# Neos-codes/microbeast

Hardware: AMD Instinct MI355X
Metric: env frames/sec (whole node) on 16x16 microRTS (higher is better)
Workload: dtype bf16

## Files before the change

### microbeast_amd/_native.py

```python
from __future__ import annotations

import ctypes
import importlib.util
import os
import sys
import threading
from pathlib import Path

import torch

_LIB = Path(__file__).resolve().parent / "_lib"
_lock = threading.Lock()
_kern = None
_rt = None

c_void_p, c_int, c_int64, c_float = ctypes.c_void_p, ctypes.c_int, ctypes.c_int64, ctypes.c_float

_SIGS = {
    "mbk_multi_copy": [c_void_p, c_int, c_void_p],
    "mbk_comm_standin": [c_void_p, c_void_p, c_int64, c_int, c_int, c_void_p],
    "mbk_row_gather": [c_void_p, c_void_p, c_void_p, c_int, c_int64, c_void_p],
    "mbk_memset": [c_void_p, c_int, c_int64, c_void_p],
    "mbk_masked_cell_fwd": [c_void_p, c_int, c_void_p, c_void_p, c_void_p, c_int, c_int64,
                            c_void_p, c_void_p, c_void_p],
    "mbk_masked_cell_bwd": [c_void_p, c_int, c_void_p, c_void_p, c_void_p, c_void_p, c_int,
                            c_int64, c_void_p, c_int, c_void_p],
    "mbk_row_sum": [c_void_p, c_int64, c_int, c_void_p, c_void_p],
    "mbk_masked_cell_fwd_pbc": [c_void_p, c_int, c_int, c_int, c_void_p, c_void_p, c_void_p,
                                c_int, c_int64, c_void_p, c_void_p, c_void_p],
    "mbk_masked_cell_bwd_pbc": [c_void_p, c_int, c_int, c_int, c_void_p, c_void_p, c_void_p,
                                c_void_p, c_int64, c_void_p, c_void_p],
    "mbk_pconv": [c_void_p, c_void_p],
    "mbk_imgconv": [c_void_p, c_int, c_void_p],
    "mbk_imgwgrad": [c_void_p, c_int, c_void_p],
    "mbk_imgwgrad_parts": [],
    "mbk_cells_nchunk": [c_int],
    "mbk_cells_compact": [c_void_p, c_int, c_int, c_int, c_void_p, c_void_p, c_void_p, c_void_p,
                          c_void_p, c_void_p, c_void_p, c_void_p, c_void_p, c_void_p],
    "mbk_rows_colsum": [c_void_p, c_int, c_int, c_void_p, c_int, c_void_p, c_void_p],
    "mbk_masked_cell_rows_fwd": [c_void_p, c_int, c_void_p, c_void_p, c_int, c_void_p, c_void_p,
                                 c_void_p, c_int, c_void_p, c_void_p, c_void_p],
    "mbk_masked_cell_rows_bwd": [c_void_p, c_int, c_void_p, c_void_p, c_int, c_int, c_void_p,
                                 c_void_p, c_void_p, c_void_p, c_void_p, c_void_p],
    "mbk_pwgrad": [c_void_p, c_void_p],
    "mbk_pwgrad_all": [c_void_p, c_void_p],
    "mbk_pwgrad_all_parts": [c_int, c_int, c_int],
    "mbk_pwgrad_parts": [c_int, c_int, c_int, c_int],
    "mbk_reduce_map": [c_void_p, c_int, c_int64, c_void_p, c_int64, c_void_p, c_void_p],
    "mbk_reduce_inv": [c_void_p, c_int, c_int64, c_void_p, c_int64, c_void_p, c_void_p, c_int64,
                       c_void_p],
    "mbk_ppool_fwd": [c_void_p, c_int, c_int, c_int, c_int, c_void_p, c_void_p, c_void_p],
    "mbk_ppool_bwd": [c_void_p, c_int64, c_int, c_void_p, c_int64, c_int, c_void_p, c_void_p,
                      c_int, c_int, c_int, c_int, c_void_p, c_void_p],
    "mbk_rng_advance": [c_void_p, c_void_p],
    "mbk_vtrace": [c_void_p, c_void_p, c_void_p, c_void_p, c_void_p, c_void_p, c_int, c_int,
                   c_float, c_float, c_float, c_float, c_float, c_float, c_float, c_void_p,
                   c_void_p, c_void_p, c_void_p, c_void_p, c_void_p, c_void_p],
    "mbk_gae": [c_void_p, c_void_p, c_void_p, c_int, c_int, c_float, c_float, c_float, c_int,
                c_void_p, c_void_p, c_void_p, c_void_p, c_void_p],
    "mbk_ppo_loss": [c_void_p, c_void_p, c_void_p, c_void_p, c_void_p, c_void_p, c_void_p,
                     c_void_p, c_int, c_int, c_float, c_float, c_float, c_float, c_float, c_float,
                     c_void_p, c_void_p, c_void_p, c_void_p, c_void_p],
    "mbk_grad_clip_scale": [c_void_p, c_int64, c_float, c_float, c_void_p, c_void_p, c_void_p],
    "mbk_adam": [c_void_p, c_void_p, c_void_p, c_void_p, c_void_p, c_int64, c_float, c_float,
                 c_float, c_float, c_float, c_int64, c_void_p, c_float, c_void_p],
    "mbk_to_bf16": [c_void_p, c_int64, c_void_p, c_void_p],
    "mbk_from_bf16": [c_void_p, c_int64, c_void_p, c_void_p],
    "mbk_conv_fwd": [c_void_p, c_int, c_int, c_int, c_void_p, c_void_p, c_void_p, c_void_p,
                     c_void_p, c_void_p, c_void_p, c_int, c_int, c_int, c_int, c_int, c_int,
                     c_void_p],
    "mbk_conv_fwd_fp8": [c_void_p, c_int, c_int, c_int, c_void_p, c_void_p, c_void_p, c_void_p,
                         c_void_p, c_int, c_int, c_int, c_int, c_int, c_int, c_void_p],
    "mbk_conv_pack_fp8": [c_void_p, c_int, c_void_p],
    "mbk_pool_bwd_idx": [c_void_p, c_void_p, c_int, c_int, c_int, c_int, c_void_p, c_void_p],
    "mbk_conv_wgrad": [c_void_p, c_int, c_int, c_int, c_void_p, c_void_p, c_void_p, c_void_p,
                       c_int, c_int, c_int, c_int, c_int, c_int, c_void_p],
    "mbk_conv_wgrad_parts": [c_int, c_int, c_int, c_int, c_int, c_int, c_int, c_int],
    "mbk_pool_conv_bwd_parts": [c_int, c_int, c_int, c_int, c_int],
    "mbk_pool_conv_bwd": [c_void_p, c_void_p, c_void_p, c_void_p, c_void_p, c_void_p, c_int,
                          c_void_p, c_void_p, c_int, c_int, c_int, c_int, c_int, c_int, c_void_p],
    "mbk_pool_conv_bwd_partial_floats": [c_int, c_int, c_int],
    "mbk_conv_set_grid_cap": [c_int],
    "mbk_set_learner_occupancy": [c_int, c_int],
    "mbk_set_work_queues": [c_int],
    "mbk_set_work_queue_site": [c_int, c_int],
    "mbk_conv0_row_set": [c_int],
    "mbk_fc_wgrad_parts": [c_int, c_int, c_int],
    "mbk_fc_wgrad": [c_void_p, c_void_p, c_int, c_int, c_int, c_void_p, c_int, c_void_p, c_int,
                     c_void_p],
    "mbk_fc_fwd": [c_void_p, c_int, c_void_p, c_void_p, c_void_p, c_void_p, c_int, c_int, c_int,
                   c_void_p, c_void_p, c_void_p],
    "mbk_gemm_nt": [c_void_p, c_void_p, c_void_p, c_void_p, c_int, c_int, c_int, c_int, c_int,
                    c_int, c_int, c_int, c_int, c_void_p],
    "mbk_wgrad_reduce": [c_void_p, c_int, c_int, c_int, c_int, c_void_p, c_void_p, c_int,
                         c_void_p],
    "mbk_wgrad_reduce_batch": [c_void_p, c_int, c_void_p],
    "mbk_pool_bwd": [c_void_p, c_void_p, c_int, c_int, c_int, c_int, c_void_p, c_void_p],
    "mbk_conv_pack": [c_void_p, c_int, c_void_p],
    "mbk_head_compact": [c_void_p, c_int, c_int, c_void_p, c_void_p, c_void_p, c_void_p,
                         c_void_p, c_void_p, c_void_p, c_void_p, c_void_p, c_void_p, c_void_p,
                         c_void_p, c_void_p, c_int, c_void_p, c_void_p, c_void_p, c_void_p],
    "mbk_head_fwd": [c_void_p, c_void_p, c_void_p, c_void_p, c_void_p, c_void_p, c_int,
                     c_void_p, c_void_p, c_void_p, c_void_p, c_void_p, c_void_p, c_int, c_int,
                     c_void_p, c_void_p, c_int, c_void_p],
    "mbk_fc_wgrad_wide_parts": [c_int, c_int, c_int],
    "mbk_fc_wgrad_wide": [c_void_p, c_void_p, c_int, c_int, c_int, c_int, c_void_p, c_int,
                          c_void_p, c_void_p, c_void_p],
    "mbk_head_score": [c_void_p, c_void_p, c_void_p, c_void_p, c_void_p, c_void_p, c_void_p,
                       c_void_p, c_void_p, c_void_p, c_void_p, c_int, c_void_p, c_void_p,
                       c_void_p, c_void_p],
    "mbk_head_pair_rowsum": [c_void_p, c_void_p, c_int, c_int, c_void_p, c_void_p, c_void_p,
                             c_void_p, c_void_p],
    "mbk_head_bwd": [c_void_p, c_void_p, c_void_p, c_void_p, c_void_p, c_void_p, c_void_p,
                     c_void_p, c_void_p, c_void_p, c_void_p, c_void_p, c_void_p, c_void_p,
                     c_void_p, c_int, c_int, c_void_p, c_void_p, c_void_p, c_void_p,
                     c_void_p, c_void_p, c_void_p],
    "mbk_head_dx_gather": [c_void_p, c_void_p, c_void_p, c_int, c_int, c_void_p, c_void_p],
    "mbk_head_dx_value_parts": [c_int],
    "mbk_head_dx_value": [c_void_p, c_void_p, c_void_p, c_int, c_int, c_void_p, c_void_p,
                          c_void_p, c_int, c_void_p, c_void_p, c_int, c_void_p],
    "mbk_head_pack": [c_void_p, c_void_p, c_int, c_void_p, c_void_p, c_void_p, c_void_p],
    "mbk_decode_obs_mask": [c_void_p, c_void_p, c_int, c_int, c_int, c_void_p, c_void_p, c_void_p],
    "mbk_decode_obs_mask_bucket": [c_void_p, c_void_p, c_int, c_int, c_int, c_void_p, c_void_p,
                                   c_void_p, c_void_p, c_void_p, c_void_p, c_void_p],
    "mbk_head_units": [c_void_p, c_int, c_int, c_void_p, c_void_p, c_void_p, c_void_p, c_void_p,
                       c_void_p],
    "mbk_row_sum_rng": [c_void_p, c_int64, c_int, c_void_p, c_void_p, c_void_p],
    "mbk_row_sum_pack": [c_void_p, c_int64, c_int, c_void_p, c_void_p, c_void_p, c_void_p,
                         c_void_p, c_int, c_void_p],
    "mbk_head_fwd_counts": [c_void_p, c_void_p, c_void_p, c_void_p, c_void_p, c_void_p,
# ... 137 lines not shown
```

### microbeast_amd/csrc/kernels/conv.hip

```cpp
#include "../include/mbk_api.h"
#include "common.h"

#include <algorithm>
#include <map>
#include <mutex>

using namespace mbk;

typedef __bf16 bf16x8 __attribute__((ext_vector_type(8)));
typedef short s16x4 __attribute__((ext_vector_type(4)));
typedef float f32x4 __attribute__((ext_vector_type(4)));
typedef __hip_bfloat16 bf16;

namespace {

constexpr int kThreads = 256;

__device__ __forceinline__ float bf2f(bf16 v) { return __bfloat162float(v); }
__device__ __forceinline__ bf16 f2bf(float v) { return __float2bfloat16(v); }

typedef short s16x2 __attribute__((ext_vector_type(2)));
__device__ __forceinline__ uint32_t relu_bf16x2(uint32_t w) {
  s16x2 v = __builtin_bit_cast(s16x2, w);
  v = __builtin_elementwise_max(v, s16x2{0, 0});
// ... 928 lines not shown
      if (tid == 0) ring[(k + 3) & 3] = gen();
      const int r0 = ring[k & 3];
      if (r0 >= nrounds) break;
      round(r0, pf0, k);
      if (tid == 0) ring[(k + 4) & 3] = gen();
      const int r1 = ring[(k + 1) & 3];
      if (r1 >= nrounds) break;
      round(r1, pf1, k + 1);
    }
    if (tid == 0 && __hip_atomic_fetch_add(wq + 1, 1, __ATOMIC_RELAXED, __HIP_MEMORY_SCOPE_AGENT) ==
                        (int)gridDim.x - 1) {
      __hip_atomic_store(wq, 0, __ATOMIC_RELAXED, __HIP_MEMORY_SCOPE_AGENT);
      __hip_atomic_store(wq + 1, 0, __ATOMIC_RELAXED, __HIP_MEMORY_SCOPE_AGENT);
    }
  } else {
    for (int rd = blockIdx.x; rd < nrounds; rd += 2 * gstep) {
      round(rd, pf0, 0);
      if (rd + gstep < nrounds) round(rd + gstep, pf1, 0);
    }
  }
  for (int w = 0; w < kThreads / 64; ++w) {
    if (wave == w) {
#pragma unroll
      for (int mb = 0; mb < MB; ++mb)
#pragma unroll
        for (int nb = 0; nb < NBLK; ++nb)
#pragma unroll
          for (int i = 0; i < 4; ++i) {
            const int co = mb * 16 + 4 * G + i, n = nb * 16 + li;
            float* p = red + co * KTOT + n;
            *p = (w == 0 ? 0.f : *p) + acc[mb][nb][i];
          }
    }
    __syncthreads();
  }
  float* out = a.partial + (size_t)blockIdx.x * (COUT * KTOT + COUT);
  for (int e = tid; e < COUT * KTOT / 4; e += kThreads) ((float4*)out)[e] = ((const float4*)red)[e];
  __syncthreads();
  float* bred = red;
  if (li == 0) {
#pragma unroll
    for (int mb = 0; mb < MB; ++mb)
#pragma unroll
      for (int i = 0; i < 4; ++i) bred[wave * COUT + mb * 16 + 4 * G + i] = accb[mb][i];
  }
  __syncthreads();
  if (tid < COUT) {
    float s = 0.f;
    for (int w = 0; w < kThreads / 64; ++w) s += bred[w * COUT + tid];
    out[COUT * KTOT + tid] = s;
  }
}

__device__ __forceinline__ void wgrad_reduce_cols(const float* __restrict__ partial, int nparts,
                                                  int pps, int split, int colblk,
                                                  float* __restrict__ stage, int cin,
                                                  int cin_real, int cout, float* __restrict__ dw,
                                                  float* __restrict__ db, int accumulate,
                                                  float (*red)[64]) {
  const int ktot = 9 * cin, row = cout * ktot + cout;
  const int col = threadIdx.x & 63, pl = threadIdx.x >> 6;
  const int e = colblk * 64 + col;
  const int p0 = split * pps, p1 = min(nparts, p0 + pps);
  float s = 0.f;
  if (e < row) {
#pragma unroll 4
    for (int p = p0 + pl; p < p1; p += 4) s += partial[(size_t)p * row + e];
  }
  red[pl][col] = s;
  __syncthreads();
  if (pl != 0 || e >= row) return;
  s = red[0][col] + red[1][col] + red[2][col] + red[3][col];
  if (stage) {
    stage[(size_t)split * row + e] = s;
    return;
  }
  if (e < cout * ktot) {
    const int co = e / ktot, r = e - co * ktot, t = r / cin, ci = r - t * cin;
    if (ci >= cin_real) return;
    float* d = dw + ((size_t)co * cin_real + ci) * 9 + t;
    *d = accumulate ? *d + s : s;
  } else if (db) {
    const int co = e - cout * ktot;
    db[co] = accumulate ? db[co] + s : s;
  }
}

__global__ __launch_bounds__(256) void wgrad_reduce_kernel(const float* __restrict__ partial,
                                                           int nparts, int pps,
                                                           float* __restrict__ stage, int cin,
                                                           int cin_real, int cout,
                                                           float* __restrict__ dw,
                                                           float* __restrict__ db, int accumulate) {
  __shared__ float red[4][64];
  wgrad_reduce_cols(partial, nparts, pps, blockIdx.y, blockIdx.x, stage, cin, cin_real, cout, dw,
                    db, accumulate, red);
}

struct MbkReduceJob {
  const float* partial;
  float* dw;
  float* db;
  int nparts, cin, cin_real, cout, accumulate;
};
constexpr int kReducePps = 32;
constexpr int kMaxReduceJobs = 32;
// ... 186 lines not shown
  const int nk = J.cin_real * 9;
  const float* wr = J.w + (size_t)co * nk;
  float m = 0.f;
  for (int e = threadIdx.x; e < nk; e += blockDim.x) m = fmaxf(m, fabsf(wr[e]));
  red[threadIdx.x] = m;
  __syncthreads();
  for (int st = 128; st > 0; st >>= 1) {
    if ((int)threadIdx.x < st) red[threadIdx.x] = fmaxf(red[threadIdx.x], red[threadIdx.x + st]);
    __syncthreads();
  }
  const float amax = red[0];
  int k = 0;
  if (amax > 0.f) {
    k = (int)floorf(log2f(224.f / amax));
    k = max(-30, min(30, k));
  }
  const float sc = ldexpf(1.f, k);
  const int nch = J.cin == 16 ? 5 : 9;
  for (int e = threadIdx.x; e < nch * 32; e += blockDim.x) {
    const int c = e / 32, kk = e % 32;
    int tap, ci;
    if (J.cin == 16) { tap = 2 * c + kk / 16; ci = kk % 16; }
    else { tap = c; ci = kk; }
    float v = 0.f;
    if (tap < 9 && ci < J.cin_real) v = wr[ci * 9 + tap] * sc;
    v = fminf(fmaxf(v, -448.f), 448.f);
    const int b = __builtin_amdgcn_cvt_pk_fp8_f32(v, 0.f, 0, false);
    J.q[(size_t)co * nch * 32 + e] = (uint8_t)(b & 0xFF);
  }
  if (threadIdx.x == 0) J.scale[co] = ldexpf(1.f, -k);
}

inline size_t fwd_smem(int cin, bool bits, int imgs, int H, int W, int cout, bool pool,
                       bool fp8 = false) {
  (void)bits;
  const int pixb = fp8 ? cin + 8 : cin * 2 + 16;
  size_t t = (((size_t)imgs * (H + 2) * (W + 2) * pixb) + 15) & ~(size_t)15;
  if (pool) t += (size_t)imgs * H * W * (cout + 4) * 2;
  return t;
}

inline size_t wgrad_smem(int cin, int cout, int imgs, int H, int W, bool unpool = false) {
  (void)unpool;
  size_t t = wg_tile_bytes(cin, cout, imgs, H, W, wg_band_w(H, W));
  t += 4096;
  t += 64;
  size_t red = (size_t)cout * 9 * cin * 4;
  return t > red ? t : red;
}

int g_grid_cap = 0;
int g_conv0_row = 1;

int resident_blocks(const void* kfn, size_t sm, int (*occ)(int) = nullptr) {
  static int cus = 0;
  if (!cus) {
    int dev = 0;
    hipGetDevice(&dev);
    hipDeviceGetAttribute(&cus, hipDeviceAttributeMultiprocessorCount, dev);
    if (cus <= 0) cus = 256;
  }
  if (sm > 64 * 1024) hipFuncSetAttribute(kfn, hipFuncAttributeMaxDynamicSharedMemorySize, (int)sm);
  int per = 0;
  if (hipOccupancyMaxActiveBlocksPerMultiprocessor(&per, kfn, kThreads, sm) != hipSuccess || per < 1)
    per = 1;
  int r = cus * (occ ? occ(per) : per);
  if (g_grid_cap > 0 && r > g_grid_cap) r = g_grid_cap;
  return r;
}

int fwd_grid(int ngroups, const void* kfn, size_t sm) {
  const long r = (long)resident_blocks(kfn, sm, mbk_occ_f);
  return (int)std::max(1L, std::min((long)ngroups, r));
}

bool index_math_ok(int imgs, int H, int W) {
  return H > 0 && W > 0 && H * W <= 1024 && (int64_t)imgs * H * W < (int64_t(1) << 22);
}

}

static int conv_fwd_launch(const void* x, int in_bits, int cin, int cout, const void* w,
                           const float* wscale, const float* bias, const void* add,
                           const void* mask_src, void* y, void* y_full, void* pool_idx, int N,
                           int H, int W, int imgs, int relu_in, int pool, bool fp8,
                           hipStream_t stream) {
  if (N <= 0) return 0;
  if (fp8 && !wscale) return (int)hipErrorInvalidValue;
  if (!index_math_ok(imgs, H, W)) return (int)hipErrorInvalidValue;
  ConvFwdArgs a{x, (const bf16*)w, bias, (const bf16*)add, (const bf16*)mask_src, (bf16*)y,
                (bf16*)y_full, (uint8_t*)pool_idx, N, H, W, imgs, relu_in, pool, wscale};
  const size_t sm = fwd_smem(cin, in_bits != 0, imgs, H, W, cout, pool != 0, fp8);
  if (sm > 160 * 1024) return (int)hipErrorInvalidValue;
  const int ngroups = (N + imgs - 1) / imgs;
#define LAUNCH(CI, CO, B)                                                                   \
  do {                                                                                      \
    auto kfn = fp8 ? conv_fwd_kernel<CI, CO, B, true> : conv_fwd_kernel<CI, CO, B, false>;  \
    if (sm > 64 * 1024) hipFuncSetAttribute((const void*)kfn,                               \
                                            hipFuncAttributeMaxDynamicSharedMemorySize, (int)sm); \
    const int grid = fwd_grid(ngroups, (const void*)kfn, sm);                               \
    hipLaunchKernelGGL(kfn, dim3(grid), dim3(kThreads), sm, stream, a);                     \
  } while (0)
  if (in_bits && cout == 16 && W > 16 && W <= 32 && !fp8 && g_conv0_row && !add && !mask_src &&
      !relu_in && kLutBytes + (size_t)kRowImgs * H * W * 16 * 2 <= 160 * 1024) {
    const size_t sm0 = kLutBytes + (pool ? (size_t)kRowImgs * H * W * 16 * 2 : 0);
    const auto kfn = conv0_row_kernel<0, 16, true>;
    const int grid = fwd_grid((N + kRowImgs - 1) / kRowImgs, (const void*)kfn, sm0);
    hipLaunchKernelGGL(kfn, dim3(grid), dim3(kThreads), sm0, stream, a);
    return (int)hipGetLastError();
  }
  if (in_bits && (cout == 16 || cout == 32) && W == 16 && !fp8 && g_conv0_row && !add &&
      !mask_src && !relu_in) {
    const size_t sm0 =
        kLutBytes + (pool ? (size_t)kRowImgs * H * 16 * conv0_ostr(cout, false) * 2 : 0);
    if (sm0 > 160 * 1024) return (int)hipErrorInvalidValue;
    const bool hb = H == 16;
    const auto kfn = cout == 16 ? (hb ? conv0_row16_kernel : conv0_row_kernel<0, 16>)
// ... 64 lines not shown
}
extern "C" int mbk_conv_wgrad_parts(int in_bits, int cin, int cout, int N, int H, int W,
                                    int imgs, int unpool) {
  const size_t sm = wgrad_smem(cin, cout, imgs, H, W, unpool != 0);
  if (sm > 160 * 1024 || !index_math_ok(imgs, H, W)) return -(int)hipErrorInvalidValue;
  const int nrounds = (N + imgs - 1) / imgs;
  int res = 1;
  const void* kq = nullptr;
#define Q(CI, CO, B) kq = wgrad_kfn<CI, CO, B>(H, W, unpool != 0)
  WGRAD_DISPATCH(Q)
#undef Q
  if (!kq) return -(int)hipErrorInvalidValue;
  res = resident_blocks(kq, sm, unpool != 0 && 2 * sm + 80 * 1024 <= 160 * 1024 ? occ_b2 : mbk_occ_b);
  return (int)std::max(1L, std::min((long)nrounds, (long)res));
}

extern "C" int mbk_conv_wgrad(const void* x, int in_bits, int cin, int cout, const void* dy,
                              const void* dp, const void* pidx, float* partial, int nparts,
                              int N, int H, int W, int imgs, int relu_in, hipStream_t stream) {
  const bool unpool = dy == nullptr;
  if (unpool && (!dp || !pidx || imgs > 2)) return (int)hipErrorInvalidValue;
  ConvWgradArgs a{x, (const bf16*)dy, partial, N, H, W, imgs, relu_in, (const bf16*)dp,
                  (const uint8_t*)pidx};
#ifndef MBK_WGRAD_QUEUE
#define MBK_WGRAD_QUEUE 1
#endif
  if (MBK_WGRAD_QUEUE) a.queue = mbk_work_queue(stream, kQueueWgrad);
  const size_t sm = wgrad_smem(cin, cout, imgs, H, W, unpool);
  if (sm > 160 * 1024 || nparts < 1 || !index_math_ok(imgs, H, W))
    return (int)hipErrorInvalidValue;
  dim3 grid(nparts);
#define LAUNCH(CI, CO, B)                                                                   \
  do {                                                                                      \
    const void* kfn = wgrad_kfn<CI, CO, B>(H, W, unpool);                    \
    if (!kfn) return (int)hipErrorInvalidValue;                              \
    if (sm > 64 * 1024)                                                                     \
      hipFuncSetAttribute(kfn, hipFuncAttributeMaxDynamicSharedMemorySize, (int)sm);        \
    void* args[] = {&a};                                                                    \
    hipLaunchKernel(kfn, grid, dim3(kThreads), args, sm, stream);                           \
  } while (0)
  if (in_bits) {
    if (cout == 16) LAUNCH(32, 16, true);
    else if (cout == 32) LAUNCH(32, 32, true);
    else return (int)hipErrorInvalidValue;
  } else if (cin == 16 && cout == 16) LAUNCH(16, 16, false);
  else if (cin == 16 && cout == 32) LAUNCH(16, 32, false);
  else if (cin == 32 && cout == 16) LAUNCH(32, 16, false);
  else if (cin == 32 && cout == 32) LAUNCH(32, 32, false);
  else return (int)hipErrorInvalidValue;
#undef LAUNCH
  return (int)hipGetLastError();
}

extern "C" void mbk_conv_set_grid_cap(int cap) { g_grid_cap = cap; }
extern "C" void mbk_conv0_row_set(int on) { g_conv0_row = on; }

extern "C" int mbk_wgrad_reduce(const float* partial, int nparts, int cin, int cin_real, int cout,
                                float* dw, float* db, int accumulate, hipStream_t stream) {
  const int row = cout * 9 * cin + cout;
  const dim3 cols((row + 63) / 64);
  if (nparts > 2 * kReducePps) {
    const int splits = (nparts + kReducePps - 1) / kReducePps;
    float* stage = (float*)partial + (size_t)nparts * row;
    hipLaunchKernelGGL(wgrad_reduce_kernel, dim3(cols.x, splits), dim3(256), 0, stream, partial,
                       nparts, kReducePps, stage, cin, cin_real, cout, dw, db, accumulate);
    hipLaunchKernelGGL(wgrad_reduce_kernel, dim3(cols.x, 1), dim3(256), 0, stream,
                       (const float*)stage, splits, splits, (float*)nullptr, cin, cin_real, cout,
                       dw, db, accumulate);
  } else {
    hipLaunchKernelGGL(wgrad_reduce_kernel, dim3(cols.x, 1), dim3(256), 0, stream, partial,
                       nparts, nparts, (float*)nullptr, cin, cin_real, cout, dw, db, accumulate);
  }
  return (int)hipGetLastError();
}

extern "C" int mbk_wgrad_reduce_batch(const MbkReduceJob* jobs, int n, hipStream_t stream) {
  for (int j0 = 0; j0 < n; j0 += kMaxReduceJobs) {
    const int nj = std::min(kMaxReduceJobs, n - j0);
    ReduceBatch b{};
    int cols = 1, splits = 1;
    bool two = false;
    for (int i = 0; i < nj; ++i) {
      const MbkReduceJob& J = jobs[j0 + i];
      if (!J.partial || !J.dw || J.nparts < 1 || J.cin < 1 || J.cout < 1 || J.cin_real > J.cin)
        return (int)hipErrorInvalidValue;
      b.j[i] = J;
      const int row = J.cout * 9 * J.cin + J.cout;
      cols = std::max(cols, (row + 63) / 64);
      if (J.nparts > 2 * kReducePps) {
        two = true;
        splits = std::max(splits, (J.nparts + kReducePps - 1) / kReducePps);
      }
    }
    hipLaunchKernelGGL(wgrad_reduce_batch_kernel, dim3(cols, splits, nj), dim3(256), 0, stream,
                       b, 0);
    if (two)
      hipLaunchKernelGGL(wgrad_reduce_batch_kernel, dim3(cols, 1, nj), dim3(256), 0, stream, b, 1);
    const int rc = (int)hipGetLastError();
    if (rc) return rc;
  }
  return 0;
}

extern "C" int mbk_pool_bwd(const void* cfull, const void* dp, int N, int H, int W, int C,
                            void* dc, hipStream_t stream) {
  const size_t tot = (size_t)N * H * W * C;
// ... 115 lines not shown
```

### microbeast_amd/ops/encoder.py

```python
from __future__ import annotations

import ctypes
from dataclasses import dataclass

import torch

from .. import _native as N
from .optim import grad_out


@dataclass
class ConvLayer:
    cin: int
    cin_real: int
    cout: int
    H: int
    W: int
    bits: bool
    relu_in: bool
    pool: bool
    w_off: int = 0
    wb_off: int = -1


class _Job(ctypes.Structure):
    _fields_ = [("w", ctypes.c_void_p), ("fwd", ctypes.c_void_p), ("bwd", ctypes.c_void_p),
                ("cin", ctypes.c_int), ("cin_real", ctypes.c_int), ("cout", ctypes.c_int)]


class _RJob(ctypes.Structure):
    _fields_ = [("partial", ctypes.c_void_p), ("dw", ctypes.c_void_p), ("db", ctypes.c_void_p),
                ("nparts", ctypes.c_int), ("cin", ctypes.c_int), ("cin_real", ctypes.c_int),
                ("cout", ctypes.c_int), ("accumulate", ctypes.c_int)]


class _Job8(ctypes.Structure):
    _fields_ = [("w", ctypes.c_void_p), ("q", ctypes.c_void_p), ("scale", ctypes.c_void_p),
                ("cin", ctypes.c_int), ("cin_real", ctypes.c_int), ("cout", ctypes.c_int)]


def _nch(c: int) -> int:
    return 5 if c == 16 else 9


_PF_FWD = 8 * 256
_PF_WGRAD = 4 * 256
_FWD_LDS = 48 * 1024
_FWD_PIX = 512
_RES32_PIX = 256
_RES32_LDS_KB = 100
_RES32_LDS_KB_SMALL = 150


def _imgs_fwd(layer: ConvLayer, cin: int, cout: int, bits: bool, pool: bool,
              fp8: bool = False) -> int:
    hw = layer.H * layer.W
    epp = 1 if bits else cin // 8
    pixb = (cin + 8) if fp8 else (cin * 2 + 16)
    imgs = max(1, _FWD_PIX // hw)
    while imgs > 1:
        sm = imgs * (layer.H + 2) * (layer.W + 2) * pixb + (imgs * hw * (cout + 4) * 2 if pool else 0)
        if sm <= _FWD_LDS and imgs * hw * epp <= _PF_FWD:
            break
        imgs //= 2
    return imgs


def _imgs_wgrad(layer: ConvLayer, unpool: bool = False, unpool_imgs: int = 2) -> int:
    hw = layer.H * layer.W
    xepp = 1 if layer.bits else layer.cin // 8
    dch = layer.cout // 8
    imgs = max(1, min(_PF_WGRAD // (hw * xepp), _PF_WGRAD // (hw * dch)))
    if layer.W in (8, 16, 24) and layer.H % 4 == 0:
        rbx = (layer.W + 2) * layer.cin * 2 + (32 if layer.cin == 32 else 64)
        rbd = layer.W * layer.cout * 2 + (32 if layer.cout == 32 else 128)
        per = (layer.H + 2) * rbx + (layer.H + (2 if layer.cin > layer.cout else 0)) * rbd
    else:
        per = (layer.H + 2) * (layer.W + 2) * layer.cin * 2 + hw * layer.cout * 2
    if unpool:
        imgs = min(imgs, unpool_imgs)
    lim = (72 if layer.cin > layer.cout else 64) * 1024
    while imgs > 1:
        if imgs * per <= lim:
            break
        imgs //= 2
    return imgs


class HipEncoder:

    def __init__(self, h: int, w: int, planes: int, channels=(16, 32, 32), device=None,
                 fp8: bool = False):
        assert planes <= 32, "bit-plane observations carry at most 32 planes"
        self.layers: list[ConvLayer] = []
        H, W, cin, cin_real, bits = h, w, 32, planes, True
        for co in channels:
            self.layers.append(ConvLayer(cin, cin_real, co, H, W, bits, False, True))
            H, W = (H + 1) // 2, (W + 1) // 2
            for _ in range(4):
                self.layers.append(ConvLayer(co, co, co, H, W, False, True, False))
            cin, cin_real, bits = co, co, False
        self.out_hw = (H, W)
        self.out_c = channels[-1]
        off = boff = 0
        for i, L in enumerate(self.layers):
            L.w_off = off
            off += L.cout * _nch(L.cin) * 32
            if i > 0:
                L.wb_off = boff
                boff += L.cin * _nch(L.cout) * 32
        self.packed_fwd = torch.zeros(off, dtype=torch.bfloat16, device=device)
        self.fused_tail = (tuple(channels) == (16, 32, 32) and self.layers[1].H <= 16
                           and self.layers[1].W <= 16)
        self.fused_res_bwd = True
        self.fused_res_bwd32 = True
        self.fused_res_fwd = True
        self.fused_res_fwd32 = True
        self.fused_stage_fwd = True
        self.fused_pool_fwd4 = True
        self.fused_res_blk32_wave = True
        self.fused_res_bwd32_team = True
        self.fused_pool_wgrad0 = True
        self.wgrad0_imgs = 1
        self.fused_pool_conv_bwd = True
        self.defer_reduce = True
        self._pbufs = {}
        self._rjobs = None
        self.packed_bwd = torch.zeros(max(boff, 1), dtype=torch.bfloat16, device=device)
        self.fp8 = fp8
        self.fused_tail8 = True
        self.packed_fwd8 = torch.zeros(off, dtype=torch.uint8, device=device)
        self.scale8 = torch.zeros(sum(L.cout for L in self.layers), dtype=torch.float32,
                                  device=device)
        self._s_off = []
        so = 0
        for L in self.layers:
            self._s_off.append(so)
            so += L.cout

    def pack(self, weights: list[torch.Tensor], with_bwd: bool) -> None:
        k = N.kernels()
        for c0 in range(0, len(self.layers), 16):
            layers = self.layers[c0:c0 + 16]
            jobs = (_Job * len(layers))()
            for i, (L, wt) in enumerate(zip(layers, weights[c0:c0 + 16])):
                assert wt.dtype == torch.float32 and wt.is_contiguous()
                bwd = ((self.packed_bwd.data_ptr() + 2 * L.wb_off)
                       if (with_bwd and L.wb_off >= 0) else None)
                jobs[i] = _Job(wt.data_ptr(), self.packed_fwd.data_ptr() + 2 * L.w_off, bwd,
                               L.cin, L.cin_real, L.cout)
            N.check(k.mbk_conv_pack(ctypes.cast(jobs, ctypes.c_void_p), len(layers),
                                    N.stream_ptr()), "conv_pack")

    def pack_layer(self, i: int, weight: torch.Tensor, with_bwd: bool = False) -> None:
        L = self.layers[i]
        assert weight.dtype == torch.float32 and weight.is_contiguous()
        bwd = ((self.packed_bwd.data_ptr() + 2 * L.wb_off)
               if (with_bwd and L.wb_off >= 0) else None)
        jobs = (_Job * 1)(_Job(weight.data_ptr(), self.packed_fwd.data_ptr() + 2 * L.w_off, bwd,
                               L.cin, L.cin_real, L.cout))
        N.check(N.kernels().mbk_conv_pack(ctypes.cast(jobs, ctypes.c_void_p), 1, N.stream_ptr()),
                "conv_pack")

    def pack_fp8(self, weights: list[torch.Tensor]) -> None:
        k = N.kernels()
        for c0 in range(0, len(self.layers), 16):
            idx = list(range(c0, min(c0 + 16, len(self.layers))))
            jobs = (_Job8 * len(idx))()
            for j, i in enumerate(idx):
                L, wt = self.layers[i], weights[i]
                assert wt.dtype == torch.float32 and wt.is_contiguous()
                jobs[j] = _Job8(wt.data_ptr(), self.packed_fwd8.data_ptr() + L.w_off,
                                self.scale8.data_ptr() + 4 * self._s_off[i], L.cin, L.cin_real,
                                L.cout)
            N.check(k.mbk_conv_pack_fp8(ctypes.cast(jobs, ctypes.c_void_p), len(idx),
# ... 34 lines not shown
                                 ctypes.cast(bp, ctypes.c_void_p), n, L1.H, L1.W,
                                 y.data_ptr(), N.stream_ptr()), "trunk_tail")
        return y

    def _tail8(self, p: torch.Tensor, bs: list[torch.Tensor]) -> torch.Tensor:
        L1, Ll = self.layers[1], self.layers[-1]
        n = p.shape[0]
        base, sbase = self.packed_fwd8.data_ptr(), self.scale8.data_ptr()
        wp = (ctypes.c_void_p * 14)(*[base + L.w_off for L in self.layers[1:15]])
        sp = (ctypes.c_void_p * 14)(*[sbase + 4 * self._s_off[i] for i in range(1, 15)])
        bp = (ctypes.c_void_p * 14)(*[b.data_ptr() for b in bs[1:15]])
        y = torch.empty(n, Ll.H, Ll.W, Ll.cout, dtype=torch.bfloat16, device=p.device)
        N.check(N.kernels().mbk_trunk_tail_fp8(
            p.data_ptr(), ctypes.cast(wp, ctypes.c_void_p), ctypes.cast(sp, ctypes.c_void_p),
            ctypes.cast(bp, ctypes.c_void_p), n, L1.H, L1.W, y.data_ptr(), N.stream_ptr()),
            "trunk_tail_fp8")
        return y

    def _fwd(self, L: ConvLayer, x, bias, add=None, mask_src=None, y_full=None, dgrad=False,
             pool_idx=None):
        n = x.shape[0]
        if dgrad:
            cin, cout, w = L.cout, L.cin, self.packed_bwd.data_ptr() + 2 * L.wb_off
            H, W = L.H, L.W
            bits, relu, pool = False, False, False
        else:
            cin, cout, w = L.cin, L.cout, self.packed_fwd.data_ptr() + 2 * L.w_off
            H, W, bits, relu, pool = L.H, L.W, L.bits, L.relu_in, L.pool
        Ho, Wo = ((H + 1) // 2, (W + 1) // 2) if pool else (H, W)
        y = torch.empty(n, Ho, Wo, cout, dtype=torch.bfloat16, device=x.device)
        imgs = _imgs_fwd(L, cin, cout, bits, pool)
        N.check(N.kernels().mbk_conv_fwd(
            x.data_ptr(), int(bits), cin, cout, w, N.ptr(bias), N.ptr(add), N.ptr(mask_src),
            y.data_ptr(), N.ptr(y_full), N.ptr(pool_idx), n, H, W, imgs, int(relu), int(pool),
            N.stream_ptr()), "conv_fwd")
        return y

    def _wgrad(self, L: ConvLayer, x, dy, dw: torch.Tensor, db: torch.Tensor, dp=None,
               pidx=None):
        n = x.shape[0]
        imgs = _imgs_wgrad(L, unpool=dy is None, unpool_imgs=self.wgrad0_imgs)
        nparts = N.kernels().mbk_conv_wgrad_parts(int(L.bits), L.cin, L.cout, n, L.H, L.W, imgs,
                                                  int(dy is None))
        if nparts < 1:
            raise RuntimeError(f"conv_wgrad: unsupported shape {L}")
        row = L.cout * 9 * L.cin + L.cout
        need = (nparts + (nparts + 31) // 32) * row
        part = self._partials(L, need, x.device)
        k = N.kernels()
        st = N.stream_ptr()
        N.check(k.mbk_conv_wgrad(x.data_ptr(), int(L.bits), L.cin, L.cout, N.ptr(dy),
                                 N.ptr(dp), N.ptr(pidx), part.data_ptr(), nparts, n,
                                 L.H, L.W, imgs, int(L.relu_in), st), "conv_wgrad")
        self._reduce(part.data_ptr(), nparts, L, dw, db)

    def _partials(self, L: ConvLayer, need: int, device) -> torch.Tensor:
        key = id(L) if self._rjobs is not None else None
        b = self._pbufs.get(key)
        if b is None or b.numel() < need or b.device != device:
            b = torch.empty(max(need, 1 << 20), dtype=torch.float32, device=device)
            self._pbufs[key] = b
        return b

    def _reduce(self, partial: int, nparts: int, L: ConvLayer, dw, db) -> None:
        job = _RJob(partial, dw.data_ptr(), db.data_ptr(), nparts, L.cin, L.cin_real, L.cout, 0)
        if self._rjobs is not None:
            self._rjobs.append(job)
            return
        N.check(N.kernels().mbk_wgrad_reduce_batch(ctypes.byref(job), 1, N.stream_ptr()),
                "wgrad_reduce_batch")

    def _flush_reduces(self) -> None:
        jobs, self._rjobs = self._rjobs, None
        if jobs:
            arr = (_RJob * len(jobs))(*jobs)
            N.check(N.kernels().mbk_wgrad_reduce_batch(ctypes.cast(arr, ctypes.c_void_p),
                                                      len(jobs), N.stream_ptr()),
                    "wgrad_reduce_batch")

    def _res_fwd16(self, li: int, p: torch.Tensor, bs: list[torch.Tensor], stage=None):
        n, H, W, C = p.shape
        outs = [torch.empty_like(p) for _ in range(4)]
        base = self.packed_fwd.data_ptr()
        wp = (ctypes.c_void_p * 4)(*[base + 2 * self.layers[li + 1 + j].w_off for j in range(4)])
        bp = (ctypes.c_void_p * 4)(*[bs[li + 1 + j].data_ptr() for j in range(4)])
        k = N.kernels()
        if stage is None:
            N.check(k.mbk_res_fwd16(p.data_ptr(), *[o.data_ptr() for o in outs],
                                    ctypes.cast(wp, ctypes.c_void_p),
                                    ctypes.cast(bp, ctypes.c_void_p), n, H, W, 4,
                                    N.stream_ptr()), "res_fwd16")
            return outs
        Ln = self.layers[li + 5]
        Ho, Wo = (H + 1) // 2, (W + 1) // 2
        pn = torch.empty(n, Ho, Wo, Ln.cout, dtype=torch.bfloat16, device=p.device)
        pidx = (torch.empty(n, Ho, Wo, Ln.cout, dtype=torch.uint8, device=p.device)
                if stage else None)
        N.check(k.mbk_res_fwd16_stage(p.data_ptr(), *[o.data_ptr() for o in outs],
                                      ctypes.cast(wp, ctypes.c_void_p),
                                      ctypes.cast(bp, ctypes.c_void_p),
                                      base + 2 * Ln.w_off, bs[li + 5].data_ptr(),
                                      pn.data_ptr(), N.ptr(pidx), n, H, W, 4,
                                      N.stream_ptr()), "res_fwd16_stage")
        return (*outs, (pn, pidx))

    def _pool_conv_fwd4(self, L: ConvLayer, x, bias, pidx):
# ... 142 lines not shown
                else:
                    u0, y0, u1, y1 = self._res_fwd16(li, p, [b.detach() for b in bs])
            elif self.fused_res_fwd32 and L.cout == 32 and p.is_cuda:
                u0, y0 = self._res_blk32(li + 1, p, bs)
                u1, y1 = self._res_blk32(li + 3, y0, bs)
            else:
                u0 = self._fwd(self.layers[li + 1], p, bs[li + 1].detach())
                y0 = self._fwd(self.layers[li + 2], u0, bs[li + 2].detach(), add=p)
                u1 = self._fwd(self.layers[li + 3], y0, bs[li + 3].detach())
                y1 = self._fwd(self.layers[li + 4], u1, bs[li + 4].detach(), add=y0)
            if save:
                saved += [x, pidx, p, u0, y0, u1]
            x = y1
            li += 5
        return x, saved

    def backward(self, g: torch.Tensor, saved: list[torch.Tensor], params: list[torch.Tensor]):
        grads = [grad_out(p) for p in params]
        nst = len(self.layers) // 5
        g = g.contiguous()
        self._rjobs = [] if self.defer_reduce and g.is_cuda else None
        for s in range(nst - 1, -1, -1):
            li = 5 * s
            x, pidx, p, u0, y0, u1 = saved[6 * s:6 * s + 6]
            L = self.layers
            if self.fused_res_bwd and L[li + 1].cin == 16 and x.is_cuda:
                dy0 = self._res_bwd16(L[li + 3], L[li + 4], y0, u1, g, grads[2 * (li + 4)],
                                      grads[2 * (li + 4) + 1], grads[2 * (li + 3)],
                                      grads[2 * (li + 3) + 1])
                dp = self._res_bwd16(L[li + 1], L[li + 2], p, u0, dy0, grads[2 * (li + 2)],
                                     grads[2 * (li + 2) + 1], grads[2 * (li + 1)],
                                     grads[2 * (li + 1) + 1])
            elif self.fused_res_bwd32 and L[li + 1].cin == 32 and x.is_cuda:
                dy0 = self._res_bwd32(L[li + 3], L[li + 4], y0, u1, g, grads[2 * (li + 4)],
                                      grads[2 * (li + 4) + 1], grads[2 * (li + 3)],
                                      grads[2 * (li + 3) + 1])
                dp = self._res_bwd32(L[li + 1], L[li + 2], p, u0, dy0, grads[2 * (li + 2)],
                                     grads[2 * (li + 2) + 1], grads[2 * (li + 1)],
                                     grads[2 * (li + 1) + 1])
            else:
                self._wgrad(L[li + 4], u1, g, grads[2 * (li + 4)], grads[2 * (li + 4) + 1])
                du1 = self._fwd(L[li + 4], g, None, mask_src=u1, dgrad=True)
                self._wgrad(L[li + 3], y0, du1, grads[2 * (li + 3)], grads[2 * (li + 3) + 1])
                dy0 = self._fwd(L[li + 3], du1, None, mask_src=y0, add=g, dgrad=True)
                self._wgrad(L[li + 2], u0, dy0, grads[2 * (li + 2)], grads[2 * (li + 2) + 1])
                du0 = self._fwd(L[li + 2], dy0, None, mask_src=u0, dgrad=True)
                self._wgrad(L[li + 1], p, du0, grads[2 * (li + 1)], grads[2 * (li + 1) + 1])
                dp = self._fwd(L[li + 1], du0, None, mask_src=p, add=dy0, dgrad=True)
            Ls = L[li]
            if (s == 0 and Ls.bits and Ls.W == 16 and self.fused_pool_wgrad0 and x.is_cuda
                    and N.kernels().mbk_conv_wgrad_parts(
                        int(Ls.bits), Ls.cin, Ls.cout, x.shape[0], Ls.H, Ls.W,
                        _imgs_wgrad(Ls, True, self.wgrad0_imgs), 1) > 0):
                self._wgrad(Ls, x, None, grads[2 * li], grads[2 * li + 1], dp=dp, pidx=pidx)
                g = None
                continue
            if (s > 0 and self.fused_pool_conv_bwd and x.is_cuda
                    and N.kernels().mbk_pool_conv_bwd_parts(x.shape[0], Ls.cin, Ls.cout, Ls.H,
                                                            Ls.W) > 0):
                g = self._pool_conv_bwd(Ls, dp, pidx, x, grads[2 * li], grads[2 * li + 1])
                continue
            dc = torch.empty(pidx.shape[0], Ls.H, Ls.W, Ls.cout, dtype=torch.bfloat16,
                             device=pidx.device)
            N.check(N.kernels().mbk_pool_bwd_idx(pidx.data_ptr(), dp.data_ptr(), pidx.shape[0],
                                                 Ls.H, Ls.W, Ls.cout, dc.data_ptr(),
                                                 N.stream_ptr()), "pool_bwd_idx")
            self._wgrad(Ls, x, dc, grads[2 * li], grads[2 * li + 1])
            g = self._fwd(Ls, dc, None, dgrad=True) if s > 0 else None
        self._flush_reduces()
        return grads


class _EncoderFn(torch.autograd.Function):
    @staticmethod
    def forward(ctx, obs_bits, enc: HipEncoder, *params):
        out, saved = enc.forward(obs_bits, list(params), save=True)
        ctx.enc = enc
        ctx.nsaved = len(saved)
        ctx.save_for_backward(*saved)
        ctx.params = params
        return out

    @staticmethod
    def backward(ctx, g):
        saved = list(ctx.saved_tensors)
        grads = ctx.enc.backward(g.to(torch.bfloat16), saved, list(ctx.params))
        return (None, None, *grads)


def encoder_params(network: torch.nn.Sequential, n_stages: int) -> list[torch.nn.Parameter]:
    out = []
    for s in range(n_stages):
        cs = network[s]
        for conv in (cs.conv, cs.res_block0.conv0, cs.res_block0.conv1, cs.res_block1.conv0,
                     cs.res_block1.conv1):
            out += [conv.weight, conv.bias]
    return out


def encode(obs_bits: torch.Tensor, enc: HipEncoder, params: list[torch.Tensor],
           need_grad: bool, prepacked: bool = False, head=None, value_out=None):
    if need_grad:
        return _EncoderFn.apply(obs_bits, enc, *params)
    with torch.no_grad():
        return enc.forward(obs_bits, [p.detach() for p in params], save=False,
                           prepacked=prepacked, head=head, value_out=value_out)[0]
```

Baseline: 19.66 million.

## Add sparse bit-packed input kernel for first-layer conv weight gradient

Adds a dedicated wave-level kernel for the first conv layer's weight gradient. It scatters the max-pool backward gradient into an LDS tile and runs MFMA only on cells whose bit-packed one-hot input differs from the empty-cell pattern. The empty-cell contribution is folded in once through an indicator-sum accumulator, so mostly-empty boards skip most of the dense work. The cost is extra per-image scatter and ballot/compaction logic, plus a new code path restricted to 16x16, 32-in, 16-out layers.

```diff
diff --git a/microbeast_amd/_native.py b/microbeast_amd/_native.py
--- a/microbeast_amd/_native.py
+++ b/microbeast_amd/_native.py
@@ -76,6 +76,9 @@
     "mbk_conv_wgrad": [c_void_p, c_int, c_int, c_int, c_void_p, c_void_p, c_void_p, c_void_p,
                        c_int, c_int, c_int, c_int, c_int, c_int, c_void_p],
     "mbk_conv_wgrad_parts": [c_int, c_int, c_int, c_int, c_int, c_int, c_int, c_int],
+    "mbk_conv_wgrad0_sparse_parts": [c_int],
+    "mbk_conv_wgrad0_sparse": [c_void_p, c_void_p, c_void_p, ctypes.c_uint, c_void_p, c_int, c_int,
+                               c_void_p],
     "mbk_pool_conv_bwd_parts": [c_int, c_int, c_int, c_int, c_int],
     "mbk_pool_conv_bwd": [c_void_p, c_void_p, c_void_p, c_void_p, c_void_p, c_void_p, c_int,
                           c_void_p, c_void_p, c_int, c_int, c_int, c_int, c_int, c_int, c_void_p],
diff --git a/microbeast_amd/csrc/kernels/conv.hip b/microbeast_amd/csrc/kernels/conv.hip
--- a/microbeast_amd/csrc/kernels/conv.hip
+++ b/microbeast_amd/csrc/kernels/conv.hip
@@ -1004,6 +1004,212 @@
   }
 }
 
+struct Wgrad0SparseArgs {
+  const uint32_t* x;
+  const bf16* dp;
+  const uint8_t* pidx;
+  float* partial;
+  int N;
+  uint32_t empty;
+  int* queue;
+};
+constexpr int kS0Waves = 3, kS0Threads = 64 * kS0Waves;
+constexpr int kS0Rbd = wg_rbd<32, 16>();
+constexpr int kS0Tile = 18 * kS0Rbd;
+constexpr int kS0WaveLds = kS0Tile + 32 * 4 + 32 * 2;
+constexpr int kS0Smem = kS0Waves * kS0WaveLds;
+static_assert(kS0WaveLds % 16 == 0 && kS0Smem >= (16 * 288 + kS0Waves * 16) * 4, "LDS carve");
+static_assert(2 * kS0Smem + 80 * 1024 <= 160 * 1024, "two workgroups beside an acting one");
+
+struct S0Img {
+  uint32_t w0, w1, w2, w3;
+  uint2 d0, d1, d2, d3;
+  uint32_t i0, i1, i2, i3;
+};
+__device__ __forceinline__ S0Img s0_load(const Wgrad0SparseArgs& a, int img, int lane) {
+  S0Img f;
+  const uint32_t* xw = a.x + (size_t)img * 256 + lane;
+  f.w0 = xw[0]; f.w1 = xw[64]; f.w2 = xw[128]; f.w3 = xw[192];
+  const int k = lane >> 2;
+  const size_t o = ((size_t)img * 64 + 16 * (k >> 2) + 2 * (k & 3)) * 16 + 4 * (lane & 3);
+  f.d0 = *(const uint2*)(a.dp + o);       f.i0 = *(const uint32_t*)(a.pidx + o);
+  f.d1 = *(const uint2*)(a.dp + o + 16);  f.i1 = *(const uint32_t*)(a.pidx + o + 16);
+  f.d2 = *(const uint2*)(a.dp + o + 128); f.i2 = *(const uint32_t*)(a.pidx + o + 128);
+  f.d3 = *(const uint2*)(a.dp + o + 144); f.i3 = *(const uint32_t*)(a.pidx + o + 144);
+  return f;
+}
+__device__ __forceinline__ void s0_scatter(char* dimg, int oy, int ox, int c0, uint2 d, uint32_t ix) {
+#pragma unroll
+  for (int j = 0; j < 4; ++j) {
+    const int t = min((int)((ix >> (8 * j)) & 0xFFu), 8);
+    const int ky = (t * 11) >> 5, kx = t - 3 * ky;
+    const int py = 2 * oy - 1 + ky, px = 2 * ox - 1 + kx;
+    uint16_t* el = (uint16_t*)(dimg + py * kS0Rbd + px * 32 + (c0 + j) * 2);
+    const uint32_t d2 = j < 2 ? d.x : d.y;
+    const float add = __uint_as_float((j & 1) ? (d2 & 0xFFFF0000u) : (d2 << 16));
+    const float v = __uint_as_float((uint32_t)*el << 16) + add;
+    *el = __bfloat16_as_ushort(f2bf(v));
+  }
+  asm volatile("" ::: "memory");
+}
+__device__ __forceinline__ uint32_t s0_pair(uint32_t x0, uint32_t x1, uint32_t bit, uint32_t k1) {
+  return ((x0 & bit) ? k1 : 0u) | ((x1 & bit) ? k1 << 16 : 0u);
+}
+
+__global__ __launch_bounds__(kS0Threads) void wgrad0_sparse_kernel(Wgrad0SparseArgs a) {
+  extern __shared__ __attribute__((aligned(16))) char smem[];
+  constexpr int RBD = kS0Rbd, DPB = 32, DIN = RBD + DPB, KTOT = 9 * 32, COUT = 16;
+  const int tid = threadIdx.x, lane = tid & 63, wave = __builtin_amdgcn_readfirstlane(tid >> 6);
+  const int G = lane >> 4, li = lane & 15;
+  char* const tile = smem + wave * kS0WaveLds;
+  uint32_t* const lw = (uint32_t*)(tile + kS0Tile);
+  uint16_t* const lp = (uint16_t*)(tile + kS0Tile + 128);
+  for (int e = lane; e < kS0WaveLds / 16; e += 64) ((uint4*)tile)[e] = make_uint4(0, 0, 0, 0);
+
+  f32x4 acc[18], accs = f32x4{0.f, 0.f, 0.f, 0.f};
+#pragma unroll
+  for (int nb = 0; nb < 18; ++nb) acc[nb] = f32x4{0.f, 0.f, 0.f, 0.f};
+  const uint32_t bit0 = 1u << li, bit1 = 1u << (li + 16);
+  const uint32_t k0 = (a.empty & bit0) ? 0xBF80u : 0x3F80u, k1 = (a.empty & bit1) ? 0xBF80u : 0x3F80u;
+  const int tky = li / 3, tkx = li - 3 * tky;
+  const uint32_t one2 = li < 9 ? 0x3F803F80u : 0u;
+  uint4 ind0 = make_uint4(one2, one2, one2, one2), ind1 = ind0;
+  if (tkx == 0) ind0.x &= 0xFFFF0000u;
+  if (tkx == 2) ind1.w &= 0x0000FFFFu;
+  const bool rowz0 = G == 0 && tky == 0, rowz3 = G == 3 && tky == 2;
+  const int sk = lane >> 2, sc0 = 4 * (lane & 3), soy = 2 * (sk >> 2), sox = 2 * (sk & 3);
+
+  auto flush = [&]() {
+    asm volatile("" ::: "memory");
+    const uint4 wa = *(const uint4*)(lw + 8 * G), wb = *(const uint4*)(lw + 8 * G + 4);
+    const char* a0 = tile + lp[8 * G + (li >> 2)] + 8 * (li & 3);
+    const char* a1 = tile + lp[8 * G + 4 + (li >> 2)] + 8 * (li & 3);
+    Frag8 b0, b1;
+    b0.u = make_uint4(s0_pair(wa.x, wa.y, bit0, k0), s0_pair(wa.z, wa.w, bit0, k0),
+                      s0_pair(wb.x, wb.y, bit0, k0), s0_pair(wb.z, wb.w, bit0, k0));
+    b1.u = make_uint4(s0_pair(wa.x, wa.y, bit1, k1), s0_pair(wa.z, wa.w, bit1, k1),
+                      s0_pair(wb.x, wb.y, bit1, k1), s0_pair(wb.z, wb.w, bit1, k1));
+#pragma unroll
+    for (int t = 0; t < 9; ++t) {
+      const int off = (2 - t / 3) * RBD + (2 - t % 3) * DPB;
+      Frag8 at;
+      at.h[0] = tr_read(a0 + off);
+      at.h[1] = tr_read(a1 + off);
+      acc[2 * t] = __builtin_amdgcn_mfma_f32_16x16x32_bf16(at.v, b0.v, acc[2 * t], 0, 0, 0);
+      acc[2 * t + 1] = __builtin_amdgcn_mfma_f32_16x16x32_bf16(at.v, b1.v, acc[2 * t + 1], 0, 0, 0);
+    }
+    asm volatile("" ::: "memory");
+  };
+  int fill = 0;
+  auto pass = [&](uint32_t w, int j) {
+    const uint32_t nz = w ^ a.empty;
+    const uint64_t m = __ballot(nz != 0u);
+    if (m == 0) return;
+    const int pre = __builtin_amdgcn_mbcnt_hi((uint32_t)(m >> 32), __builtin_amdgcn_mbcnt_lo((uint32_t)m, 0u));
+    int slot = nz != 0u ? fill + pre : -1;
+    int total = fill + __popcll(m);
+    const int cell = 64 * j + lane;
+    const uint16_t off = (uint16_t)((cell >> 4) * RBD + (cell & 15) * DPB);
+    for (;;) {
+      if (slot >= 0 && slot < 32) {
+        lw[slot] = nz;
+        lp[slot] = off;
+      }
+      if (total < 32) break;
+      flush();
+      slot -= 32;
+      total -= 32;
+    }
+    fill = total;
+  };
+
+  const int nwaves = (int)gridDim.x * kS0Waves;
+  int cend = 0;
+  int img = a.queue ? mbk::wave_next_item(a.queue, -1, cend, a.N) : (int)blockIdx.x * kS0Waves + wave;
+  img = __builtin_amdgcn_readfirstlane(img);
+  S0Img nx{};
+  if (img < a.N) nx = s0_load(a, img, lane);
+  while (img < a.N) {
+    const S0Img cu = nx;
+    int nimg = a.queue ? mbk::wave_next_item(a.queue, img, cend, a.N) : img + nwaves;
+    nimg = __builtin_amdgcn_readfirstlane(nimg);
+    if (nimg < a.N) nx = s0_load(a, nimg, lane);
+#pragma unroll
+    for (int i = 0; i < 8; ++i) {
+      const int e = lane + 64 * i;
+      *(uint4*)(tile + DIN + (e >> 5) * RBD + (e & 31) * 16) = make_uint4(0, 0, 0, 0);
+    }
+    asm volatile("" ::: "memory");
+    s0_scatter(tile + DIN, soy, sox, sc0, cu.d0, cu.i0);
+    s0_scatter(tile + DIN, soy, sox + 1, sc0, cu.d1, cu.i1);
+    s0_scatter(tile + DIN, soy + 1, sox, sc0, cu.d2, cu.i2);
+    s0_scatter(tile + DIN, soy + 1, sox + 1, sc0, cu.d3, cu.i3);
+#pragma unroll
+    for (int b = 0; b < 4; ++b)
+#pragma unroll
+      for (int c = 0; c < 2; ++c) {
+        const char* db = tile + DIN + (4 * b + G) * RBD + (8 * c + (li >> 2)) * DPB + 8 * (li & 3);
+        Frag8 at, in;
+        at.h[0] = tr_read(db);
+        at.h[1] = tr_read(db + 4 * DPB);
+        in.u = c ? ind1 : ind0;
+        if ((b == 0 && rowz0) || (b == 3 && rowz3)) in.u = make_uint4(0, 0, 0, 0);
+        accs = __builtin_amdgcn_mfma_f32_16x16x32_bf16(at.v, in.v, accs, 0, 0, 0);
+      }
+    pass(cu.w0, 0);
+    pass(cu.w1, 1);
+    pass(cu.w2, 2);
+    pass(cu.w3, 3);
+    if (fill > 0) {
+      if (lane >= fill && lane < 32) {
+        lw[lane] = 0u;
+        lp[lane] = (uint16_t)(17 * DPB);
+      }
+      flush();
+      fill = 0;
+    }
+    img = nimg;
+  }
+  if (a.queue) mbk::wave_queue_done(a.queue, nwaves);
+
+  const float e0 = (a.empty & bit0) ? 1.f : 0.f, e1 = (a.empty & bit1) ? 1.f : 0.f;
+#pragma unroll
+  for (int t = 0; t < 9; ++t)
+#pragma unroll
+    for (int i = 0; i < 4; ++i) {
+      const float s = __shfl(accs[i], 16 * G + t, 64);
+      acc[2 * t][i] += e0 * s;
+      acc[2 * t + 1][i] += e1 * s;
+    }
+  __syncthreads();
+  float* red = (float*)smem;
+  for (int w = 0; w < kS0Waves; ++w) {
+    if (wave == w) {
+#pragma unroll
+      for (int nb = 0; nb < 18; ++nb)
+#pragma unroll
+        for (int i = 0; i < 4; ++i) {
+          float* p = red + (4 * G + i) * KTOT + nb * 16 + li;
+          *p = (w == 0 ? 0.f : *p) + acc[nb][i];
+        }
+    }
+    __syncthreads();
+  }
+  float* bred = red + COUT * KTOT;
+  if (li == 4) {
+#pragma unroll
+    for (int i = 0; i < 4; ++i) bred[wave * COUT + 4 * G + i] = accs[i];
+  }
+  __syncthreads();
+  float* out = a.partial + (size_t)blockIdx.x * (COUT * KTOT + COUT);
+  for (int e = tid; e < COUT * KTOT / 4; e += kS0Threads) ((float4*)out)[e] = ((const float4*)red)[e];
+  if (tid < COUT) {
+    float s = 0.f;
+    for (int w = 0; w < kS0Waves; ++w) s += bred[w * COUT + tid];
+    out[COUT * KTOT + tid] = s;
+  }
+}
+
 __device__ __forceinline__ void wgrad_reduce_cols(const float* __restrict__ partial, int nparts,
                                                   int pps, int split, int colblk,
                                                   float* __restrict__ stage, int cin,
@@ -1296,7 +1502,7 @@
 int g_grid_cap = 0;
 int g_conv0_row = 1;
 
-int resident_blocks(const void* kfn, size_t sm, int (*occ)(int) = nullptr) {
+int resident_blocks(const void* kfn, size_t sm, int (*occ)(int) = nullptr, int threads = kThreads) {
   static int cus = 0;
   if (!cus) {
     int dev = 0;
@@ -1306,7 +1512,7 @@
   }
   if (sm > 64 * 1024) hipFuncSetAttribute(kfn, hipFuncAttributeMaxDynamicSharedMemorySize, (int)sm);
   int per = 0;
-  if (hipOccupancyMaxActiveBlocksPerMultiprocessor(&per, kfn, kThreads, sm) != hipSuccess || per < 1)
+  if (hipOccupancyMaxActiveBlocksPerMultiprocessor(&per, kfn, threads, sm) != hipSuccess || per < 1)
     per = 1;
   int r = cus * (occ ? occ(per) : per);
   if (g_grid_cap > 0 && r > g_grid_cap) r = g_grid_cap;
@@ -1477,6 +1683,23 @@
   return (int)hipGetLastError();
 }
 
+extern "C" int mbk_conv_wgrad0_sparse_parts(int N) {
+  if (N < 1) return -(int)hipErrorInvalidValue;
+  const int res = resident_blocks((const void*)wgrad0_sparse_kernel, kS0Smem, occ_b2, kS0Threads);
+  return (int)std::max(1L, std::min((long)(N + kS0Waves - 1) / kS0Waves, (long)res));
+}
+
+extern "C" int mbk_conv_wgrad0_sparse(const void* x, const void* dp, const void* pidx,
+                                      unsigned empty_word, float* partial, int nparts, int N,
+                                      hipStream_t stream) {
+  if (!x || !dp || !pidx || !partial || nparts < 1 || N < 1) return (int)hipErrorInvalidValue;
+  Wgrad0SparseArgs a{(const uint32_t*)x, (const bf16*)dp, (const uint8_t*)pidx, partial, N,
+                     empty_word, nullptr};
+  if (MBK_WGRAD_QUEUE) a.queue = mbk_work_queue(stream, kQueueWgrad);
+  hipLaunchKernelGGL(wgrad0_sparse_kernel, dim3(nparts), dim3(kS0Threads), kS0Smem, stream, a);
+  return (int)hipGetLastError();
+}
+
 extern "C" void mbk_conv_set_grid_cap(int cap) { g_grid_cap = cap; }
 extern "C" void mbk_conv0_row_set(int on) { g_conv0_row = on; }
 
diff --git a/microbeast_amd/ops/encoder.py b/microbeast_amd/ops/encoder.py
--- a/microbeast_amd/ops/encoder.py
+++ b/microbeast_amd/ops/encoder.py
@@ -42,6 +42,9 @@
 def _nch(c: int) -> int:
     return 5 if c == 16 else 9
 
+
+PLANE_GROUPS = ((0, 5), (5, 5), (10, 3), (13, 8), (21, 6))
+EMPTY_WORD = sum(1 << off for off, _ in PLANE_GROUPS)
 
 _PF_FWD = 8 * 256
 _PF_WGRAD = 4 * 256
@@ -121,6 +124,7 @@
         self.fused_res_blk32_wave = True
         self.fused_res_bwd32_team = True
         self.fused_pool_wgrad0 = True
+        self.sparse_wgrad0 = True
         self.wgrad0_imgs = 1
         self.fused_pool_conv_bwd = True
         self.defer_reduce = True
@@ -261,6 +265,20 @@
         N.check(k.mbk_conv_wgrad(x.data_ptr(), int(L.bits), L.cin, L.cout, N.ptr(dy),
                                  N.ptr(dp), N.ptr(pidx), part.data_ptr(), nparts, n,
                                  L.H, L.W, imgs, int(L.relu_in), st), "conv_wgrad")
+        self._reduce(part.data_ptr(), nparts, L, dw, db)
+
+    def _wgrad0_sparse(self, L: ConvLayer, x, dp, pidx, dw: torch.Tensor, db: torch.Tensor):
+        n = x.shape[0]
+        k = N.kernels()
+        nparts = k.mbk_conv_wgrad0_sparse_parts(n)
+        if nparts < 1:
+            raise RuntimeError(f"conv_wgrad0_sparse: unsupported batch {n}")
+        row = L.cout * 9 * L.cin + L.cout
+        need = (nparts + (nparts + 31) // 32) * row
+        part = self._partials(L, need, x.device)
+        N.check(k.mbk_conv_wgrad0_sparse(x.data_ptr(), dp.data_ptr(), pidx.data_ptr(), EMPTY_WORD,
+                                         part.data_ptr(), nparts, n, N.stream_ptr()),
+                "conv_wgrad0_sparse")
         self._reduce(part.data_ptr(), nparts, L, dw, db)
 
     def _partials(self, L: ConvLayer, need: int, device) -> torch.Tensor:
@@ -509,7 +527,10 @@
                     and N.kernels().mbk_conv_wgrad_parts(
                         int(Ls.bits), Ls.cin, Ls.cout, x.shape[0], Ls.H, Ls.W,
                         _imgs_wgrad(Ls, True, self.wgrad0_imgs), 1) > 0):
-                self._wgrad(Ls, x, None, grads[2 * li], grads[2 * li + 1], dp=dp, pidx=pidx)
+                if self.sparse_wgrad0 and (Ls.H, Ls.cin, Ls.cout) == (16, 32, 16):
+                    self._wgrad0_sparse(Ls, x, dp, pidx, grads[2 * li], grads[2 * li + 1])
+                else:
+                    self._wgrad(Ls, x, None, grads[2 * li], grads[2 * li + 1], dp=dp, pidx=pidx)
                 g = None
                 continue
             if (s > 0 and self.fused_pool_conv_bwd and x.is_cuda
```

New measurement: 20.96 million (median of 6 runs). 1.07x the previous value.
